# petuum/autodist

Hardware: AMD Instinct MI355X
Metric: images/sec ResNet-50 AllReduce (higher is better)
Workload: dtype bf16; 1 GPU; model=resnet50, global_batch=512, parallelism=dp1, image_size=224

## Files before the change

### autodist_amd/models/resnet.py

```python
import torch
import torch.nn as nn


def _make_bn(ch, fused, relu):
    if fused:
        from autodist_amd.ops.fused_bn import FusedBatchNorm2d
        return FusedBatchNorm2d(ch, relu=relu)
    return nn.BatchNorm2d(ch)


class Bottleneck(nn.Module):
    expansion = 4

    def __init__(self, in_ch, width, stride=1, downsample=None, fused=False):
        super().__init__()
        out_ch = width * self.expansion
        self.fused = fused
        self.conv1 = nn.Conv2d(in_ch, width, 1, bias=False)
        self.bn1 = _make_bn(width, fused, relu=True)
        self.conv2 = nn.Conv2d(width, width, 3, stride=stride, padding=1,
                               bias=False)
        self.bn2 = _make_bn(width, fused, relu=True)
        self.conv3 = nn.Conv2d(width, out_ch, 1, bias=False)
        self.bn3 = _make_bn(out_ch, fused, relu=True)
        self.relu = nn.ReLU(inplace=True)
        self.downsample = downsample

    def forward(self, x):
        if self.fused:
            out = self.bn1(self.conv1(x))
            out = self.bn2(self.conv2(out))
            z = self.conv3(out)
            identity = x if self.downsample is None else self.downsample(x)
            return self.bn3.forward_add(z, identity)
        identity = x
        out = self.relu(self.bn1(self.conv1(x)))
        out = self.relu(self.bn2(self.conv2(out)))
        out = self.bn3(self.conv3(out))
        if self.downsample is not None:
            identity = self.downsample(x)
        return self.relu(out + identity)


class BasicBlock(nn.Module):
    expansion = 1

    def __init__(self, in_ch, width, stride=1, downsample=None, fused=False):
        super().__init__()
        self.fused = fused
        self.conv1 = nn.Conv2d(in_ch, width, 3, stride=stride, padding=1,
                               bias=False)
        self.bn1 = _make_bn(width, fused, relu=True)
        self.conv2 = nn.Conv2d(width, width, 3, padding=1, bias=False)
        self.bn2 = _make_bn(width, fused, relu=True)
        self.relu = nn.ReLU(inplace=True)
        self.downsample = downsample

    def forward(self, x):
        if self.fused:
            out = self.bn1(self.conv1(x))
            z = self.conv2(out)
            identity = x if self.downsample is None else self.downsample(x)
            return self.bn2.forward_add(z, identity)
        identity = x
        out = self.relu(self.bn1(self.conv1(x)))
        out = self.bn2(self.conv2(out))
        if self.downsample is not None:
            identity = self.downsample(x)
        return self.relu(out + identity)


class ResNet(nn.Module):
    def __init__(self, block, layers, num_classes=1000, fused=False):
        super().__init__()
        self.in_ch = 64
        self.fused = fused
        self.conv1 = nn.Conv2d(3, 64, 7, stride=2, padding=3, bias=False)
        self.bn1 = _make_bn(64, fused, relu=True)
# ... 17 lines not shown
    def _make_layer(self, block, width, blocks, stride=1):
        downsample = None
        out_ch = width * block.expansion
        if stride != 1 or self.in_ch != out_ch:
            downsample = nn.Sequential(
                nn.Conv2d(self.in_ch, out_ch, 1, stride=stride, bias=False),
                _make_bn(out_ch, self.fused, relu=False))
        layers = [block(self.in_ch, width, stride, downsample,
                        fused=self.fused)]
        self.in_ch = out_ch
        for _ in range(1, blocks):
            layers.append(block(self.in_ch, width, fused=self.fused))
        return nn.Sequential(*layers)

    def forward(self, x):
        x = self.bn1(self.conv1(x))
        if not self.fused:
            x = self.relu(x)
        x = self.maxpool(x)
        x = self.layer4(self.layer3(self.layer2(self.layer1(x))))
        x = self.avgpool(x).flatten(1)
        return self.fc(x)


def resnet18(num_classes=1000, fused=False):
    return ResNet(BasicBlock, [2, 2, 2, 2], num_classes, fused=fused)


def resnet50(num_classes=1000, fused=False):
    return ResNet(Bottleneck, [3, 4, 6, 3], num_classes, fused=fused)


def resnet101(num_classes=1000, fused=False):
    return ResNet(Bottleneck, [3, 4, 23, 3], num_classes, fused=fused)
# ... 1 lines not shown
```

### autodist_amd/ops/csrc/bn_ops.hip

```cpp
#include "common.h"

#define BN_VEC 8
#define BN_RED_U 4
#define BN_FIN_U 8
#define BN_RELU_NONE 0
#define BN_RELU_Y 1
#define BN_RELU_MASK 2

__device__ __forceinline__ void load8(const __hip_bfloat16* p, float* v) {
  const __hip_bfloat162* p2 = reinterpret_cast<const __hip_bfloat162*>(p);
  float2 a = __bfloat1622float2(p2[0]);
  float2 b = __bfloat1622float2(p2[1]);
  float2 c = __bfloat1622float2(p2[2]);
  float2 d = __bfloat1622float2(p2[3]);
  v[0] = a.x; v[1] = a.y; v[2] = b.x; v[3] = b.y;
  v[4] = c.x; v[5] = c.y; v[6] = d.x; v[7] = d.y;
}
__device__ __forceinline__ void store8(__hip_bfloat16* p, const float* v) {
  __hip_bfloat162* p2 = reinterpret_cast<__hip_bfloat162*>(p);
  p2[0] = __float22bfloat162_rn({v[0], v[1]});
  p2[1] = __float22bfloat162_rn({v[2], v[3]});
  p2[2] = __float22bfloat162_rn({v[4], v[5]});
  p2[3] = __float22bfloat162_rn({v[6], v[7]});
}
// ... 43 lines not shown
                                        float* v) {
  const unsigned w[4] = {r.a.x, r.a.y, r.a.z, r.a.w};
#pragma unroll
  for (int j = 0; j < 4; ++j) {
    v[2 * j] = __uint_as_float(w[j] << 16);
    v[2 * j + 1] = __uint_as_float(w[j] & 0xffff0000u);
  }
}
__device__ __forceinline__ void unpack8(const Raw8<float>& r, float* v) {
  v[0] = r.a.x; v[1] = r.a.y; v[2] = r.a.z; v[3] = r.a.w;
  v[4] = r.b.x; v[5] = r.b.y; v[6] = r.b.z; v[7] = r.b.w;
}
__device__ __forceinline__ void apply_mask8(unsigned bits, float* dv) {
#pragma unroll
  for (int k = 0; k < BN_VEC; ++k) dv[k] = (bits >> k) & 1u ? dv[k] : 0.f;
}

template <typename T>
__global__ void __launch_bounds__(BLOCK_THREADS)
bn_fwd_reduce_kernel(const T* __restrict__ x, float* __restrict__ partial_sum,
                     float* __restrict__ partial_sq, long M, int C) {
#pragma clang fp contract(off)
  int tx_count = min(C / BN_VEC, (int)blockDim.x);
  int tx = threadIdx.x % tx_count;
  int ty = threadIdx.x / tx_count;
  int rows_per_blk = blockDim.x / tx_count;
  int c0 = (blockIdx.y * tx_count + tx) * BN_VEC;
  if (c0 >= C) return;
  float s[BN_VEC] = {0}, q[BN_VEC] = {0};
  const long stride = (long)gridDim.x * rows_per_blk;
// ... 134 lines not shown
#pragma unroll
      for (int k = 0; k < BN_VEC; ++k) v[k] += r[k];
    }
    if (RELU) {
#pragma unroll
      for (int k = 0; k < BN_VEC; ++k) v[k] = fmaxf(v[k], 0.f);
    }
    if (MASK)
      mask[m * (C / BN_VEC) + c0 / BN_VEC] =
          (unsigned char)store8_mask(y + m * C + c0, v);
    else
      store8(y + m * C + c0, v);
  }
}

template <typename T, int RELU>
__device__ __forceinline__ void bn_load_dz(const T* __restrict__ dy,
                                           const T* __restrict__ y,
                                           const unsigned char* __restrict__ mask,
                                           long m, int C, int c0, float* dv) {
  load8(dy + m * C + c0, dv);
  if (RELU == BN_RELU_Y) {
    float yv[BN_VEC];
    load8(y + m * C + c0, yv);
#pragma unroll
    for (int k = 0; k < BN_VEC; ++k) dv[k] = yv[k] > 0.f ? dv[k] : 0.f;
  }
  if (RELU == BN_RELU_MASK)
    apply_mask8(mask[m * (C / BN_VEC) + c0 / BN_VEC], dv);
}

template <typename T, int RELU>
__global__ void __launch_bounds__(BLOCK_THREADS)
bn_bwd_reduce_kernel(const T* __restrict__ x, const T* __restrict__ dy,
                     const T* __restrict__ y,
                     const unsigned char* __restrict__ mask,
                     const float* __restrict__ save_mean,
                     const float* __restrict__ save_rstd,
                     float* __restrict__ partial_dz,
                     float* __restrict__ partial_dzxh, long M, int C) {
#pragma clang fp contract(off)
  int tx_count = min(C / BN_VEC, (int)blockDim.x);
  int tx = threadIdx.x % tx_count;
  int ty = threadIdx.x / tx_count;
  int rows_per_blk = blockDim.x / tx_count;
  int c0 = (blockIdx.y * tx_count + tx) * BN_VEC;
  if (c0 >= C) return;
  float mean[BN_VEC], rstd[BN_VEC];
  load8(save_mean + c0, mean);
  load8(save_rstd + c0, rstd);
  float s[BN_VEC] = {0}, t[BN_VEC] = {0};
  const long stride = (long)gridDim.x * rows_per_blk;
  long m = (long)blockIdx.x * rows_per_blk + ty;
  for (; m + (BN_RED_U - 1) * stride < M; m += BN_RED_U * stride) {
    Raw8<T> rx[BN_RED_U], rd[BN_RED_U], ry[BN_RED_U];
    unsigned rm[BN_RED_U];
#pragma unroll
    for (int u = 0; u < BN_RED_U; ++u) {
      const long mu = m + u * stride;
      rx[u] = load8raw(x + mu * C + c0);
      rd[u] = load8raw(dy + mu * C + c0);
      if (RELU == BN_RELU_Y) ry[u] = load8raw(y + mu * C + c0);
      if (RELU == BN_RELU_MASK) rm[u] = mask[mu * (C / BN_VEC) + c0 / BN_VEC];
    }
    __builtin_amdgcn_sched_barrier(0);
#pragma unroll
    for (int u = 0; u < BN_RED_U; ++u) {
      float xv[BN_VEC], dv[BN_VEC];
      unpack8(rx[u], xv);
      unpack8(rd[u], dv);
      if (RELU == BN_RELU_Y) {
        float yv[BN_VEC];
        unpack8(ry[u], yv);
#pragma unroll
        for (int k = 0; k < BN_VEC; ++k) dv[k] = yv[k] > 0.f ? dv[k] : 0.f;
      }
      if (RELU == BN_RELU_MASK) apply_mask8(rm[u], dv);
#pragma unroll
      for (int k = 0; k < BN_VEC; ++k) {
        s[k] += dv[k];
        t[k] = fmaf(dv[k] * (xv[k] - mean[k]), rstd[k], t[k]);
      }
    }
  }
  for (; m < M; m += stride) {
    float xv[BN_VEC], dv[BN_VEC];
    load8(x + m * C + c0, xv);
    bn_load_dz<T, RELU>(dy, y, mask, m, C, c0, dv);
#pragma unroll
    for (int k = 0; k < BN_VEC; ++k) {
      s[k] += dv[k];
      t[k] = fmaf(dv[k] * (xv[k] - mean[k]), rstd[k], t[k]);
    }
  }
  __shared__ float ls[BLOCK_THREADS * BN_VEC];
  __shared__ float lt[BLOCK_THREADS * BN_VEC];
#pragma unroll
  for (int k = 0; k < BN_VEC; ++k) {
    ls[threadIdx.x * BN_VEC + k] = s[k];
    lt[threadIdx.x * BN_VEC + k] = t[k];
  }
  __syncthreads();
  if (ty == 0) {
// ... 40 lines not shown
  dweight[c] = sdzxh;
  dbias[c] = sdz;
}

template <typename T, int RELU, bool ADD>
__global__ void bn_bwd_apply_kernel(const T* __restrict__ x,
                                    const T* __restrict__ dy,
                                    const T* __restrict__ y,
                                    const unsigned char* __restrict__ mask,
                                    const float* __restrict__ save_mean,
                                    const float* __restrict__ save_rstd,
                                    const float* __restrict__ k1,
                                    const float* __restrict__ k2,
                                    const float* __restrict__ k3,
                                    T* __restrict__ dx, T* __restrict__ dres,
                                    long M, int C) {
  int tx_count = min(C / BN_VEC, (int)blockDim.x);
  int tx = threadIdx.x % tx_count;
  int ty = threadIdx.x / tx_count;
  int rows_per_blk = blockDim.x / tx_count;
  int c0 = (blockIdx.y * tx_count + tx) * BN_VEC;
  if (c0 >= C) return;
  float mean[BN_VEC], rstd[BN_VEC], a1[BN_VEC], a2[BN_VEC], a3[BN_VEC];
  load8(save_mean + c0, mean);
  load8(save_rstd + c0, rstd);
  load8(k1 + c0, a1);
  load8(k2 + c0, a2);
  load8(k3 + c0, a3);
  for (long m = (long)blockIdx.x * rows_per_blk + ty; m < M;
       m += (long)gridDim.x * rows_per_blk) {
    float xv[BN_VEC], dv[BN_VEC];
    load8(x + m * C + c0, xv);
    bn_load_dz<T, RELU>(dy, y, mask, m, C, c0, dv);
    if (ADD) store8(dres + m * C + c0, dv);
    float o[BN_VEC];
#pragma unroll
    for (int k = 0; k < BN_VEC; ++k) {
      float xhat = (xv[k] - mean[k]) * rstd[k];
      o[k] = a1[k] * (dv[k] - a2[k] - xhat * a3[k]);
    }
    store8(dx + m * C + c0, o);
  }
}
```

### autodist_amd/ops/csrc/ext.hip

```cpp
#include <torch/extension.h>
#include <ATen/cuda/CUDAContext.h>

#include "multi_tensor.hip"
#include "bn_ops.hip"
#include "psgd_gemm.hip"
#include "mfma_probe.hip"
#include "attention.hip"
#include "attention_bwd.hip"
#include "ln_ops.hip"
#include "ce_ops.hip"

namespace {

inline hipStream_t cur_stream() {
  return at::cuda::getCurrentCUDAStream().stream();
}

struct BNGeom {
  long M;
  int C;
  int tx_count, rows_per_blk, grid_c;
};

BNGeom bn_geom(const torch::Tensor& x) {
// ... 32 lines not shown
T* bn_ptr(const torch::Tensor& t) {
  return reinterpret_cast<T*>(t.data_ptr());
}

template <typename T, bool RELU, bool ADD, bool MASK>
void bn_launch_fwd_apply(dim3 grid, hipStream_t st, const torch::Tensor& x,
                         const torch::Tensor* res, torch::Tensor& y,
                         unsigned char* mask, const float* scale,
                         const float* shift, const BNGeom& g) {
  hipLaunchKernelGGL((bn_fwd_apply_kernel<T, RELU, ADD, MASK>), grid,
                     dim3(BLOCK_THREADS), 0, st, bn_ptr<const T>(x),
                     ADD ? bn_ptr<const T>(*res) : (const T*)nullptr,
                     bn_ptr<T>(y), mask, scale, shift, g.M, g.C);
}

template <typename T>
std::vector<torch::Tensor> bn_fwd_impl(
    const torch::Tensor& x, const torch::Tensor& weight,
    const torch::Tensor& bias, torch::Tensor& running_mean,
    torch::Tensor& running_var, const c10::optional<torch::Tensor>& res,
    double eps, double momentum, bool relu,
    const c10::optional<torch::Tensor>& ws, bool with_mask) {
  TORCH_CHECK(!with_mask || relu, "the mask is the ReLU mask: relu must be set");
  auto g = bn_geom(x);
  auto fopt = weight.options().dtype(torch::kFloat32);
  torch::Tensor w6 = ws.has_value() ? *ws
      : torch::empty({2 * BN_GM_MAX + 4, (long)g.C}, fopt);
  TORCH_CHECK(w6.size(0) >= 2 * BN_GM_MAX + 4 && w6.size(1) == g.C &&
              w6.is_contiguous());
  float* wp = w6.data_ptr<float>();
  float* partial_sum = wp;
  float* partial_sq = wp + (long)BN_GM_MAX * g.C;
  auto stats = torch::empty({2, (long)g.C}, fopt);
  auto save_mean = stats[0];
  auto save_rstd = stats[1];
  torch::Tensor mask;
  if (with_mask)
    mask = torch::empty({g.M, (long)(g.C / BN_VEC)},
                        x.options().dtype(torch::kUInt8));
  unsigned char* mp = with_mask ? mask.data_ptr<unsigned char>() : nullptr;
  const float* scale = wp + (long)(2 * BN_GM_MAX + 2) * g.C;
  const float* shift = wp + (long)(2 * BN_GM_MAX + 3) * g.C;
  auto y = torch::empty_like(x);
  int gm = bn_reduce_gm(g);
  dim3 grid_r(gm, g.grid_c);
  dim3 grid_a(bn_grid_m(g, 4096), g.grid_c);
  auto st = cur_stream();

  hipLaunchKernelGGL((bn_fwd_reduce_kernel<T>), grid_r, dim3(BLOCK_THREADS),
                     0, st, bn_ptr<const T>(x), partial_sum, partial_sq, g.M,
                     g.C);
  hipLaunchKernelGGL(bn_fwd_finalize_kernel,
                     dim3((g.C + FIN_CH - 1) / FIN_CH),
                     dim3(FIN_CH * FIN_LANES), 0, st, partial_sum, partial_sq,
                     gm, weight.data_ptr<float>(), bias.data_ptr<float>(),
                     running_mean.data_ptr<float>(),
                     running_var.data_ptr<float>(),
                     save_mean.data_ptr<float>(), save_rstd.data_ptr<float>(),
                     const_cast<float*>(scale), const_cast<float*>(shift),
                     g.M, g.C, (float)eps, (float)momentum);
  const torch::Tensor* rp = res.has_value() ? &*res : nullptr;
#define BN_FWD_APPLY(RELU, ADD, MASK)                                        \
  bn_launch_fwd_apply<T, RELU, ADD, MASK>(grid_a, st, x, rp, y, mp, scale,  \
                                          shift, g)
  if (rp) {
    if (with_mask) BN_FWD_APPLY(true, true, true);
    else if (relu) BN_FWD_APPLY(true, true, false);
    else BN_FWD_APPLY(false, true, false);
  } else {
    if (with_mask) BN_FWD_APPLY(true, false, true);
    else if (relu) BN_FWD_APPLY(true, false, false);
    else BN_FWD_APPLY(false, false, false);
  }
#undef BN_FWD_APPLY
  if (with_mask) return {y, save_mean, save_rstd, mask};
// ... 22 lines not shown
                                        c10::optional<torch::Tensor> res,
                                        double eps, double momentum,
                                        bool relu,
                                        c10::optional<torch::Tensor> ws) {
  return bn_fwd_dispatch(x, weight, bias, running_mean, running_var, res, eps,
                         momentum, relu, ws, false);
}

std::vector<torch::Tensor> bn_fwd_train_mask(
    torch::Tensor x, torch::Tensor weight, torch::Tensor bias,
    torch::Tensor running_mean, torch::Tensor running_var,
    c10::optional<torch::Tensor> res, double eps, double momentum, bool relu,
    c10::optional<torch::Tensor> ws) {
  return bn_fwd_dispatch(x, weight, bias, running_mean, running_var, res, eps,
                         momentum, relu, ws, true);
}

template <typename T, int RELU>
std::vector<torch::Tensor> bn_bwd_impl(
    const torch::Tensor& x, const torch::Tensor& dy, const torch::Tensor& yq,
    const torch::Tensor& save_mean, const torch::Tensor& save_rstd,
    const torch::Tensor& weight, bool need_dres,
    const c10::optional<torch::Tensor>& ws) {
  auto g = bn_geom(x);
  auto fopt = weight.options().dtype(torch::kFloat32);
  torch::Tensor w5 = ws.has_value() ? *ws
      : torch::empty({2 * BN_GM_MAX + 3, (long)g.C}, fopt);
  TORCH_CHECK(w5.size(0) >= 2 * BN_GM_MAX + 3 && w5.size(1) == g.C &&
              w5.is_contiguous());
  const T* yp = nullptr;
// ... 16 lines not shown
  auto dweight = torch::empty({g.C}, fopt);
  auto dbias = torch::empty({g.C}, fopt);
  auto dx = torch::empty_like(x);
  torch::Tensor dres;
  if (need_dres) dres = torch::empty_like(x);
  dim3 block(BLOCK_THREADS);
  int gm = bn_reduce_gm(g);
  dim3 grid_r(gm, g.grid_c);
  dim3 grid_a(bn_grid_m(g, 4096), g.grid_c);
  auto st = cur_stream();
  const float* sm = save_mean.data_ptr<float>();
  const float* sr = save_rstd.data_ptr<float>();

  hipLaunchKernelGGL((bn_bwd_reduce_kernel<T, RELU>), grid_r, block, 0, st,
                     bn_ptr<const T>(x), bn_ptr<const T>(dy), yp, mp, sm, sr,
                     partial_dz, partial_dzxh, g.M, g.C);
  hipLaunchKernelGGL(bn_bwd_finalize_kernel,
                     dim3((g.C + FIN_CH - 1) / FIN_CH),
                     dim3(FIN_CH * FIN_LANES), 0, st, partial_dz,
                     partial_dzxh, gm, weight.data_ptr<float>(), sr, k1, k2,
                     k3, dweight.data_ptr<float>(), dbias.data_ptr<float>(),
                     g.M, g.C);
  if (need_dres)
    hipLaunchKernelGGL((bn_bwd_apply_kernel<T, RELU, true>), grid_a, block, 0,
                       st, bn_ptr<const T>(x), bn_ptr<const T>(dy), yp, mp,
                       sm, sr, k1, k2, k3, bn_ptr<T>(dx), bn_ptr<T>(dres),
                       g.M, g.C);
  else
    hipLaunchKernelGGL((bn_bwd_apply_kernel<T, RELU, false>), grid_a, block,
                       0, st, bn_ptr<const T>(x), bn_ptr<const T>(dy), yp, mp,
                       sm, sr, k1, k2, k3, bn_ptr<T>(dx), (T*)nullptr, g.M,
                       g.C);
  std::vector<torch::Tensor> out = {dx, dweight, dbias};
  if (need_dres) out.push_back(dres);
  return out;
}

template <int RELU>
std::vector<torch::Tensor> bn_bwd_dispatch(
    const torch::Tensor& x, const torch::Tensor& dy, const torch::Tensor& yq,
    const torch::Tensor& save_mean, const torch::Tensor& save_rstd,
    const torch::Tensor& weight, bool need_dres,
    const c10::optional<torch::Tensor>& ws) {
  if (x.scalar_type() == torch::kBFloat16)
    return bn_bwd_impl<__hip_bfloat16, RELU>(x, dy, yq, save_mean, save_rstd,
                                             weight, need_dres, ws);
  TORCH_CHECK(x.scalar_type() == torch::kFloat32);
// ... 12 lines not shown
                                      need_dres, ws);
  return bn_bwd_dispatch<BN_RELU_NONE>(x, dy, y, save_mean, save_rstd, weight,
                                       need_dres, ws);
}

std::vector<torch::Tensor> bn_bwd_mask(torch::Tensor x, torch::Tensor dy,
                                       torch::Tensor mask,
                                       torch::Tensor save_mean,
                                       torch::Tensor save_rstd,
                                       torch::Tensor weight, bool relu,
                                       bool need_dres,
                                       c10::optional<torch::Tensor> ws) {
  TORCH_CHECK(relu, "the mask is the ReLU mask: relu must be set");
  return bn_bwd_dispatch<BN_RELU_MASK>(x, dy, mask, save_mean, save_rstd,
                                       weight, need_dres, ws);
}

void check_f32_flat(const torch::Tensor& t, const char* name) {
  TORCH_CHECK(t.is_cuda(), name, " must be on GPU");
  TORCH_CHECK(t.is_contiguous(), name, " must be contiguous");
  TORCH_CHECK(t.scalar_type() == torch::kFloat32, name, " must be fp32");
}

template <typename GT>
void launch_fused_sgd(torch::Tensor& p, const GT* g,
                      c10::optional<torch::Tensor>& buf, double lr,
                      double momentum, double dampening, double weight_decay,
                      bool nesterov, bool first_step, bool maximize) {
  long n = p.numel();
  dim3 grid(grid_for(n)), block(BLOCK_THREADS);
// ... 656 lines not shown
  m.def("scatter_add_rows", &scatter_add_rows, "rowwise scatter-add");
  m.def("gather_rows", &gather_rows, "rowwise gather");
  m.def("sparse_apply_rows", &sparse_apply_rows,
        "fused row-wise SGD/Adagrad/Adam update of unique rows (gfx950)");
  m.def("bn_fwd_train", &bn_fwd_train,
        "fused NHWC batchnorm fwd (+add+relu), returns y/save_mean/save_rstd");
  m.def("bn_bwd", &bn_bwd,
        "fused NHWC batchnorm bwd (+relu-mask+dres), returns "
        "dx/dweight/dbias[/dres]");
  m.def("bn_fwd_train_mask", &bn_fwd_train_mask,
        "bn_fwd_train with relu that also returns the bit-packed ReLU mask "
        "[M, C/8] uint8");
  m.def("bn_bwd_mask", &bn_bwd_mask,
        "bn_bwd that takes the packed mask of bn_fwd_train_mask in place of "
        "y");
  m.attr("BN_RED_U") = BN_RED_U;
  m.attr("BN_FIN_U") = BN_FIN_U;
  m.def("psgd_mq", &psgd_mq, "PowerSGD P = M @ Q (MFMA f32 16x16x4)");
  m.def("psgd_mtp", &psgd_mtp, "PowerSGD Qn = M^T @ P (MFMA f32 16x16x4)");
  m.def("psgd_decompress_ef", &psgd_decompress_ef,
        "fused hat = P Q^T * scale; err = M - hat; flat = hat");
  m.def("psgd_add_err_pad", &psgd_add_err_pad,
        "padded M = flat + err (zero tail)");
  m.def("mfma_probe", &mfma_probe,
        "diagnostic: v_mfma_f32_16x16x32_bf16 A/B layout probe");
  m.def("ce_fwd", &ce_fwd,
        "fused online-softmax cross-entropy fwd -> loss_rows, m, l2s");
  m.def("ce_bwd", &ce_bwd, "fused cross-entropy bwd -> dlogits (bf16)");
  m.def("col_sum", &col_sum, "bf16 [N,H] column sum -> fp32 [H]");
  m.def("ln_fwd", &ln_fwd,
// ... 18 lines not shown
```

### autodist_amd/ops/fused_bn.py

```python
from typing import Optional

import torch

from autodist_amd.ops import api as ops_api


class _FusedBNFunction(torch.autograd.Function):
    @staticmethod
    def forward(ctx, x, weight, bias, running_mean, running_var,
                momentum, eps, relu, residual, ws=None):
        use_hip = x.is_cuda and ops_api.has_gpu_ops()
        ctx.ws_bwd = ws[1] if ws is not None else None
        if use_hip and relu:
            y, save_mean, save_rstd, sign = ops_api.ext().bn_fwd_train_mask(
                x, weight, bias, running_mean, running_var, residual,
                eps, momentum, relu, ws[0] if ws is not None else None)
        elif use_hip:
            y, save_mean, save_rstd = ops_api.ext().bn_fwd_train(
                x, weight, bias, running_mean, running_var, residual,
                eps, momentum, relu, ws[0] if ws is not None else None)
            sign = y
        else:
            xf = x.float()
            m = xf.numel() // xf.size(1)
# ... 31 lines not shown
                weight, relu, has_res, ctx.ws_bwd)
            dx, dweight, dbias = out[0], out[1], out[2]
            dres = out[3] if has_res else None
        else:
            dyf = dy.float()
            if relu:
                dyf = dyf * (sign > 0).float()
            dres = dyf.to(dy.dtype) if has_res else None
            dxf, dweight, dbias = torch.ops.aten.native_batch_norm_backward(
                dyf, x.float(), weight, None, None, save_mean, save_rstd,
                True, 0.0, [True, True, True])
            dx = dxf.to(x.dtype)
        return (dx, dweight, dbias, None, None, None, None, None, dres, None)


def fused_bn_train(x, weight, bias, running_mean, running_var,
                   momentum=0.1, eps=1e-5, relu=False,
                   residual: Optional[torch.Tensor] = None, ws=None):
    return _FusedBNFunction.apply(x, weight, bias, running_mean, running_var,
                                  momentum, eps, relu, residual, ws)


class FusedBatchNorm2d(torch.nn.Module):

    def __init__(self, num_features, eps=1e-5, momentum=0.1, relu=False):
        super().__init__()
        self.num_features = num_features
        self.eps = eps
        self.momentum = momentum
        self.relu = relu
        self.weight = torch.nn.Parameter(torch.ones(num_features))
        self.bias = torch.nn.Parameter(torch.zeros(num_features))
        self.register_buffer("running_mean", torch.zeros(num_features))
        self.register_buffer("running_var", torch.ones(num_features))
        self.register_buffer("num_batches_tracked",
                             torch.tensor(0, dtype=torch.long))
        self._ws = None

    def _check(self, x):
        if x.is_cuda and not x.is_contiguous(memory_format=torch.channels_last):
            x = x.contiguous(memory_format=torch.channels_last)
        return x

    def forward(self, x, residual: Optional[torch.Tensor] = None):
        x = self._check(x)
        if residual is not None:
            residual = self._check(residual)
        if self.training:
            self.num_batches_tracked += 1
            if x.is_cuda and (self._ws is None
                              or self._ws[0].device != x.device):
                self._ws = (
                    torch.empty(2 * 512 + 4, self.num_features,
                                device=x.device),
                    torch.empty(2 * 512 + 3, self.num_features,
                                device=x.device))
            return fused_bn_train(x, self.weight, self.bias,
                                  self.running_mean, self.running_var,
                                  self.momentum, self.eps, self.relu, residual,
                                  ws=self._ws if x.is_cuda else None)
        scale = self.weight * (self.running_var + self.eps).rsqrt()
        shift = self.bias - self.running_mean * scale
        y = x * scale[None, :, None, None].to(x.dtype) + \
            shift[None, :, None, None].to(x.dtype)
        if residual is not None:
            y = y + residual
        return torch.relu(y) if self.relu else y

    def forward_add(self, x, residual):
        return self.forward(x, residual)

    def extra_repr(self):
        return f"{self.num_features}, relu={self.relu}"
```

Before: 9384 images/sec.

## Fuse stem BN+ReLU+maxpool and downsample BN into residual BN apply

Adds a fused kernel for the stem that applies BN, ReLU and the 3x3 stride-2 max-pool in one pass, storing packed argmax words instead of the full-resolution activation. The backward pass recomputes the pooled gradient scatter inside the BN backward reduce and apply kernels. It also fuses the downsample-branch BN into the residual-add BN apply, so the downsample BN output is never materialized. This cuts full-size activation writes and reads and some launches, at the cost of more complex gather logic and bf16 rounding-order subtleties.

New measurement: 9898 images/sec (median of 6 runs). +5.5%, better.

```diff
diff --git a/autodist_amd/models/resnet.py b/autodist_amd/models/resnet.py
--- a/autodist_amd/models/resnet.py
+++ b/autodist_amd/models/resnet.py
@@ -31,8 +31,10 @@
             out = self.bn1(self.conv1(x))
             out = self.bn2(self.conv2(out))
             z = self.conv3(out)
-            identity = x if self.downsample is None else self.downsample(x)
-            return self.bn3.forward_add(z, identity)
+            if self.downsample is None:
+                return self.bn3.forward_add(z, x)
+            return self.bn3.forward_add_bn(z, self.downsample[0](x),
+                                           self.downsample[1])
         identity = x
         out = self.relu(self.bn1(self.conv1(x)))
         out = self.relu(self.bn2(self.conv2(out)))
@@ -60,8 +62,10 @@
         if self.fused:
             out = self.bn1(self.conv1(x))
             z = self.conv2(out)
-            identity = x if self.downsample is None else self.downsample(x)
-            return self.bn2.forward_add(z, identity)
+            if self.downsample is None:
+                return self.bn2.forward_add(z, x)
+            return self.bn2.forward_add_bn(z, self.downsample[0](x),
+                                           self.downsample[1])
         identity = x
         out = self.relu(self.bn1(self.conv1(x)))
         out = self.bn2(self.conv2(out))
@@ -109,10 +113,10 @@
         return nn.Sequential(*layers)
 
     def forward(self, x):
-        x = self.bn1(self.conv1(x))
-        if not self.fused:
-            x = self.relu(x)
-        x = self.maxpool(x)
+        if self.fused:
+            x = self.bn1.forward_pool(self.conv1(x))
+        else:
+            x = self.maxpool(self.relu(self.bn1(self.conv1(x))))
         x = self.layer4(self.layer3(self.layer2(self.layer1(x))))
         x = self.avgpool(x).flatten(1)
         return self.fc(x)
diff --git a/autodist_amd/ops/csrc/bn_ops.hip b/autodist_amd/ops/csrc/bn_ops.hip
--- a/autodist_amd/ops/csrc/bn_ops.hip
+++ b/autodist_amd/ops/csrc/bn_ops.hip
@@ -81,6 +81,65 @@
 __device__ __forceinline__ void apply_mask8(unsigned bits, float* dv) {
 #pragma unroll
   for (int k = 0; k < BN_VEC; ++k) dv[k] = (bits >> k) & 1u ? dv[k] : 0.f;
+}
+
+__device__ __forceinline__ float round_to(float v, const __hip_bfloat16*) {
+  return __bfloat162float(__float2bfloat16(v));
+}
+__device__ __forceinline__ float round_to(float v, const float*) { return v; }
+
+#define BN_RELU_POOL 3
+#define BN_POOL_NONE 15u
+#define BN_POOL_NEVER 14u
+struct BNPool {
+  const unsigned* amax;
+  int H, W, Ho, Wo;
+};
+template <typename T>
+struct PoolTaps {
+  Raw8<T> d[4];
+  unsigned a[4];
+  unsigned codes;
+};
+template <typename T>
+__device__ __forceinline__ void pool_issue(const T* __restrict__ dy,
+                                           const BNPool& p, long m, int C,
+                                           int c0, PoolTaps<T>& t) {
+  const unsigned mm = (unsigned)m;
+  const unsigned q = mm / (unsigned)p.W;
+  const int w = (int)(mm - q * (unsigned)p.W);
+  const unsigned n = q / (unsigned)p.H;
+  const int h = (int)(q - n * (unsigned)p.H);
+  const int ho = h >> 1, wo = w >> 1;
+  const bool hb = (h & 1) && ho + 1 < p.Ho;
+  const bool wb = (w & 1) && wo + 1 < p.Wo;
+  const unsigned kh = 1 + (h & 1), kw = 1 + (w & 1);
+  const unsigned o0 = ((n * p.Ho + ho) * p.Wo + wo) * C + c0;
+  const unsigned dh = hb ? p.Wo * C : 0, dw = wb ? C : 0;
+  const unsigned o[4] = {o0, o0 + dw, o0 + dh, o0 + dh + dw};
+  t.codes = (kh * 3 + kw) | (wb ? kh * 3 : BN_POOL_NEVER) << 8 |
+            (hb ? kw : BN_POOL_NEVER) << 16 |
+            (hb && wb ? 0u : BN_POOL_NEVER) << 24;
+#pragma unroll
+  for (int j = 0; j < 4; ++j) {
+    t.d[j] = load8raw(dy + o[j]);
+    t.a[j] = p.amax[o[j] / BN_VEC];
+  }
+}
+template <typename T>
+__device__ __forceinline__ void pool_dz(const PoolTaps<T>& t, float* dv) {
+  float acc[BN_VEC] = {0};
+#pragma unroll
+  for (int j = 0; j < 4; ++j) {
+    float d[BN_VEC];
+    unpack8(t.d[j], d);
+    const unsigned e = t.a[j] ^ (((t.codes >> (8 * j)) & 15u) * 0x11111111u);
+#pragma unroll
+    for (int k = 0; k < BN_VEC; ++k)
+      acc[k] += ((e >> (4 * k)) & 15u) == 0u ? d[k] : 0.f;
+  }
+#pragma unroll
+  for (int k = 0; k < BN_VEC; ++k) dv[k] = round_to(acc[k], (const T*)nullptr);
 }
 
 template <typename T>
@@ -245,11 +304,115 @@
   }
 }
 
+template <typename T>
+__global__ void bn_fwd_pool_apply_kernel(const T* __restrict__ x,
+                                         T* __restrict__ y,
+                                         unsigned* __restrict__ amax,
+                                         const float* __restrict__ scale,
+                                         const float* __restrict__ shift,
+                                         BNPool p, long Mo, int C) {
+  int tx_count = min(C / BN_VEC, (int)blockDim.x);
+  int tx = threadIdx.x % tx_count;
+  int ty = threadIdx.x / tx_count;
+  int rows_per_blk = blockDim.x / tx_count;
+  int c0 = (blockIdx.y * tx_count + tx) * BN_VEC;
+  if (c0 >= C) return;
+  float sc[BN_VEC], sh[BN_VEC];
+  load8(scale + c0, sc);
+  load8(shift + c0, sh);
+  for (long mo = (long)blockIdx.x * rows_per_blk + ty; mo < Mo;
+       mo += (long)gridDim.x * rows_per_blk) {
+    const unsigned mm = (unsigned)mo;
+    const unsigned q = mm / (unsigned)p.Wo;
+    const int wo = (int)(mm - q * (unsigned)p.Wo);
+    const unsigned n = q / (unsigned)p.Ho;
+    const int ho = (int)(q - n * (unsigned)p.Ho);
+    Raw8<T> rx[9];
+    bool ok[9];
+#pragma unroll
+    for (int kh = 0; kh < 3; ++kh) {
+      const int h = 2 * ho - 1 + kh;
+      const int hc = min(max(h, 0), p.H - 1);
+#pragma unroll
+      for (int kw = 0; kw < 3; ++kw) {
+        const int w = 2 * wo - 1 + kw;
+        const int wc = min(max(w, 0), p.W - 1);
+        ok[kh * 3 + kw] = h == hc && w == wc;
+        rx[kh * 3 + kw] =
+            load8raw(x + (((long)n * p.H + hc) * p.W + wc) * C + c0);
+      }
+    }
+    float best[BN_VEC];
+    unsigned idx[BN_VEC];
+#pragma unroll
+    for (int k = 0; k < BN_VEC; ++k) { best[k] = -1.f; idx[k] = 0; }
+#pragma unroll
+    for (int j = 0; j < 9; ++j) {
+      float v[BN_VEC];
+      unpack8(rx[j], v);
+#pragma unroll
+      for (int k = 0; k < BN_VEC; ++k) {
+        float r = round_to(fmaxf(fmaf(v[k], sc[k], sh[k]), 0.f),
+                           (const T*)nullptr);
+        const bool take = ok[j] && r > best[k];
+        best[k] = take ? r : best[k];
+        idx[k] = take ? (unsigned)j : idx[k];
+      }
+    }
+    unsigned word = 0;
+#pragma unroll
+    for (int k = 0; k < BN_VEC; ++k)
+      word |= (best[k] > 0.f ? idx[k] : BN_POOL_NONE) << (4 * k);
+    store8(y + mo * C + c0, best);
+    amax[mo * (C / BN_VEC) + c0 / BN_VEC] = word;
+  }
+}
+
+template <typename T>
+__global__ void bn_fwd_apply_add_bn_kernel(
+    const T* __restrict__ z, const T* __restrict__ zd, T* __restrict__ y,
+    unsigned char* __restrict__ mask, const float* __restrict__ scale,
+    const float* __restrict__ shift, const float* __restrict__ scale_d,
+    const float* __restrict__ shift_d, long M, int C) {
+  int tx_count = min(C / BN_VEC, (int)blockDim.x);
+  int tx = threadIdx.x % tx_count;
+  int ty = threadIdx.x / tx_count;
+  int rows_per_blk = blockDim.x / tx_count;
+  int c0 = (blockIdx.y * tx_count + tx) * BN_VEC;
+  if (c0 >= C) return;
+  float sc[BN_VEC], sh[BN_VEC], scd[BN_VEC], shd[BN_VEC];
+  load8(scale + c0, sc);
+  load8(shift + c0, sh);
+  load8(scale_d + c0, scd);
+  load8(shift_d + c0, shd);
+  for (long m = (long)blockIdx.x * rows_per_blk + ty; m < M;
+       m += (long)gridDim.x * rows_per_blk) {
+    float v[BN_VEC], r[BN_VEC];
+    load8(z + m * C + c0, v);
+    load8(zd + m * C + c0, r);
+#pragma unroll
+    for (int k = 0; k < BN_VEC; ++k) {
+      v[k] = fmaf(v[k], sc[k], sh[k]);
+      v[k] += round_to(fmaf(r[k], scd[k], shd[k]), (const T*)nullptr);
+      v[k] = fmaxf(v[k], 0.f);
+    }
+    mask[m * (C / BN_VEC) + c0 / BN_VEC] =
+        (unsigned char)store8_mask(y + m * C + c0, v);
+  }
+}
+
 template <typename T, int RELU>
 __device__ __forceinline__ void bn_load_dz(const T* __restrict__ dy,
                                            const T* __restrict__ y,
                                            const unsigned char* __restrict__ mask,
-                                           long m, int C, int c0, float* dv) {
+                                           const BNPool& pool, long m, int C,
+                                           int c0, float* dv) {
+  if (RELU == BN_RELU_POOL) {
+    PoolTaps<T> t;
+    pool_issue(dy, pool, m, C, c0, t);
+    pool_dz(t, dv);
+    return;
+  }
   load8(dy + m * C + c0, dv);
   if (RELU == BN_RELU_Y) {
     float yv[BN_VEC];
@@ -263,13 +426,15 @@
 
 template <typename T, int RELU>
 __global__ void __launch_bounds__(BLOCK_THREADS)
+__attribute__((amdgpu_waves_per_eu(RELU == BN_RELU_POOL ? 2 : 1)))
 bn_bwd_reduce_kernel(const T* __restrict__ x, const T* __restrict__ dy,
                      const T* __restrict__ y,
                      const unsigned char* __restrict__ mask,
                      const float* __restrict__ save_mean,
                      const float* __restrict__ save_rstd,
                      float* __restrict__ partial_dz,
-                     float* __restrict__ partial_dzxh, long M, int C) {
+                     float* __restrict__ partial_dzxh, long M, int C,
+                     BNPool pool) {
 #pragma clang fp contract(off)
   int tx_count = min(C / BN_VEC, (int)blockDim.x);
   int tx = threadIdx.x % tx_count;
@@ -286,11 +451,17 @@
   for (; m + (BN_RED_U - 1) * stride < M; m += BN_RED_U * stride) {
     Raw8<T> rx[BN_RED_U], rd[BN_RED_U], ry[BN_RED_U];
     unsigned rm[BN_RED_U];
+    PoolTaps<T> rp[BN_RED_U];
 #pragma unroll
     for (int u = 0; u < BN_RED_U; ++u) {
       const long mu = m + u * stride;
       rx[u] = load8raw(x + mu * C + c0);
-      rd[u] = load8raw(dy + mu * C + c0);
+      if (RELU == BN_RELU_POOL) {
+        pool_issue(dy, pool, mu, C, c0, rp[u]);
+        __builtin_amdgcn_sched_barrier(0);
+      } else {
+        rd[u] = load8raw(dy + mu * C + c0);
+      }
       if (RELU == BN_RELU_Y) ry[u] = load8raw(y + mu * C + c0);
       if (RELU == BN_RELU_MASK) rm[u] = mask[mu * (C / BN_VEC) + c0 / BN_VEC];
     }
@@ -299,7 +470,8 @@
     for (int u = 0; u < BN_RED_U; ++u) {
       float xv[BN_VEC], dv[BN_VEC];
       unpack8(rx[u], xv);
-      unpack8(rd[u], dv);
+      if (RELU == BN_RELU_POOL) pool_dz(rp[u], dv);
+      else unpack8(rd[u], dv);
       if (RELU == BN_RELU_Y) {
         float yv[BN_VEC];
         unpack8(ry[u], yv);
@@ -312,12 +484,13 @@
         s[k] += dv[k];
         t[k] = fmaf(dv[k] * (xv[k] - mean[k]), rstd[k], t[k]);
       }
+      if (RELU == BN_RELU_POOL) __builtin_amdgcn_sched_barrier(0);
     }
   }
   for (; m < M; m += stride) {
     float xv[BN_VEC], dv[BN_VEC];
     load8(x + m * C + c0, xv);
-    bn_load_dz<T, RELU>(dy, y, mask, m, C, c0, dv);
+    bn_load_dz<T, RELU>(dy, y, mask, pool, m, C, c0, dv);
 #pragma unroll
     for (int k = 0; k < BN_VEC; ++k) {
       s[k] += dv[k];
@@ -388,7 +561,7 @@
                                     const float* __restrict__ k2,
                                     const float* __restrict__ k3,
                                     T* __restrict__ dx, T* __restrict__ dres,
-                                    long M, int C) {
+                                    long M, int C, BNPool pool) {
   int tx_count = min(C / BN_VEC, (int)blockDim.x);
   int tx = threadIdx.x % tx_count;
   int ty = threadIdx.x / tx_count;
@@ -405,7 +578,7 @@
        m += (long)gridDim.x * rows_per_blk) {
     float xv[BN_VEC], dv[BN_VEC];
     load8(x + m * C + c0, xv);
-    bn_load_dz<T, RELU>(dy, y, mask, m, C, c0, dv);
+    bn_load_dz<T, RELU>(dy, y, mask, pool, m, C, c0, dv);
     if (ADD) store8(dres + m * C + c0, dv);
     float o[BN_VEC];
 #pragma unroll
diff --git a/autodist_amd/ops/csrc/ext.hip b/autodist_amd/ops/csrc/ext.hip
--- a/autodist_amd/ops/csrc/ext.hip
+++ b/autodist_amd/ops/csrc/ext.hip
@@ -70,15 +70,19 @@
                      bn_ptr<T>(y), mask, scale, shift, g.M, g.C);
 }
 
+struct BNStats {
+  torch::Tensor save_mean, save_rstd;
+  const float* scale;
+  const float* shift;
+  torch::Tensor ws;
+};
+
 template <typename T>
-std::vector<torch::Tensor> bn_fwd_impl(
-    const torch::Tensor& x, const torch::Tensor& weight,
-    const torch::Tensor& bias, torch::Tensor& running_mean,
-    torch::Tensor& running_var, const c10::optional<torch::Tensor>& res,
-    double eps, double momentum, bool relu,
-    const c10::optional<torch::Tensor>& ws, bool with_mask) {
-  TORCH_CHECK(!with_mask || relu, "the mask is the ReLU mask: relu must be set");
-  auto g = bn_geom(x);
+BNStats bn_fwd_stats(const torch::Tensor& x, const BNGeom& g,
+                     const torch::Tensor& weight, const torch::Tensor& bias,
+                     torch::Tensor& running_mean, torch::Tensor& running_var,
+                     double eps, double momentum,
+                     const c10::optional<torch::Tensor>& ws) {
   auto fopt = weight.options().dtype(torch::kFloat32);
   torch::Tensor w6 = ws.has_value() ? *ws
       : torch::empty({2 * BN_GM_MAX + 4, (long)g.C}, fopt);
@@ -90,17 +94,10 @@
   auto stats = torch::empty({2, (long)g.C}, fopt);
   auto save_mean = stats[0];
   auto save_rstd = stats[1];
-  torch::Tensor mask;
-  if (with_mask)
-    mask = torch::empty({g.M, (long)(g.C / BN_VEC)},
-                        x.options().dtype(torch::kUInt8));
-  unsigned char* mp = with_mask ? mask.data_ptr<unsigned char>() : nullptr;
   const float* scale = wp + (long)(2 * BN_GM_MAX + 2) * g.C;
   const float* shift = wp + (long)(2 * BN_GM_MAX + 3) * g.C;
-  auto y = torch::empty_like(x);
   int gm = bn_reduce_gm(g);
   dim3 grid_r(gm, g.grid_c);
-  dim3 grid_a(bn_grid_m(g, 4096), g.grid_c);
   auto st = cur_stream();
 
   hipLaunchKernelGGL((bn_fwd_reduce_kernel<T>), grid_r, dim3(BLOCK_THREADS),
@@ -115,6 +112,31 @@
                      save_mean.data_ptr<float>(), save_rstd.data_ptr<float>(),
                      const_cast<float*>(scale), const_cast<float*>(shift),
                      g.M, g.C, (float)eps, (float)momentum);
+  return {save_mean, save_rstd, scale, shift, w6};
+}
+
+template <typename T>
+std::vector<torch::Tensor> bn_fwd_impl(
+    const torch::Tensor& x, const torch::Tensor& weight,
+    const torch::Tensor& bias, torch::Tensor& running_mean,
+    torch::Tensor& running_var, const c10::optional<torch::Tensor>& res,
+    double eps, double momentum, bool relu,
+    const c10::optional<torch::Tensor>& ws, bool with_mask) {
+  TORCH_CHECK(!with_mask || relu, "the mask is the ReLU mask: relu must be set");
+  auto g = bn_geom(x);
+  BNStats s = bn_fwd_stats<T>(x, g, weight, bias, running_mean, running_var,
+                              eps, momentum, ws);
+  auto save_mean = s.save_mean, save_rstd = s.save_rstd;
+  const float* scale = s.scale;
+  const float* shift = s.shift;
+  torch::Tensor mask;
+  if (with_mask)
+    mask = torch::empty({g.M, (long)(g.C / BN_VEC)},
+                        x.options().dtype(torch::kUInt8));
+  unsigned char* mp = with_mask ? mask.data_ptr<unsigned char>() : nullptr;
+  auto y = torch::empty_like(x);
+  dim3 grid_a(bn_grid_m(g, 4096), g.grid_c);
+  auto st = cur_stream();
   const torch::Tensor* rp = res.has_value() ? &*res : nullptr;
 #define BN_FWD_APPLY(RELU, ADD, MASK)                                        \
   bn_launch_fwd_apply<T, RELU, ADD, MASK>(grid_a, st, x, rp, y, mp, scale,  \
@@ -167,6 +189,107 @@
     c10::optional<torch::Tensor> ws) {
   return bn_fwd_dispatch(x, weight, bias, running_mean, running_var, res, eps,
                          momentum, relu, ws, true);
+}
+
+inline BNPool bn_pool_geom(const torch::Tensor& x, const BNGeom& g) {
+  BNPool p;
+  p.amax = nullptr;
+  p.H = (int)x.size(2);
+  p.W = (int)x.size(3);
+  p.Ho = (p.H - 1) / 2 + 1;
+  p.Wo = (p.W - 1) / 2 + 1;
+  TORCH_CHECK(g.M < (1L << 31), "bn pool: N*H*W must be below 2^31");
+  TORCH_CHECK(x.size(0) * (long)p.Ho * p.Wo * g.C < (1L << 31),
+              "bn pool: the pooled tensor must hold fewer than 2^31 elements");
+  return p;
+}
+
+template <typename T>
+std::vector<torch::Tensor> bn_fwd_pool_impl(
+    const torch::Tensor& x, const torch::Tensor& weight,
+    const torch::Tensor& bias, torch::Tensor& running_mean,
+    torch::Tensor& running_var, double eps, double momentum,
+    const c10::optional<torch::Tensor>& ws) {
+  auto g = bn_geom(x);
+  BNPool p = bn_pool_geom(x, g);
+  BNStats s = bn_fwd_stats<T>(x, g, weight, bias, running_mean, running_var,
+                              eps, momentum, ws);
+  BNGeom go = g;
+  go.M = x.size(0) * (long)p.Ho * p.Wo;
+  auto y = torch::empty({x.size(0), x.size(1), (long)p.Ho, (long)p.Wo},
+                        x.options().memory_format(at::MemoryFormat::ChannelsLast));
+  auto amax = torch::empty({go.M, (long)(g.C / BN_VEC)},
+                           x.options().dtype(torch::kInt32));
+  dim3 grid_a(bn_grid_m(go, 4096), g.grid_c);
+  hipLaunchKernelGGL((bn_fwd_pool_apply_kernel<T>), grid_a,
+                     dim3(BLOCK_THREADS), 0, cur_stream(), bn_ptr<const T>(x),
+                     bn_ptr<T>(y), bn_ptr<unsigned>(amax), s.scale, s.shift,
+                     p, go.M, g.C);
+  return {y, s.save_mean, s.save_rstd, amax};
+}
+
+std::vector<torch::Tensor> bn_fwd_train_pool(
+    torch::Tensor x, torch::Tensor weight, torch::Tensor bias,
+    torch::Tensor running_mean, torch::Tensor running_var, double eps,
+    double momentum, c10::optional<torch::Tensor> ws) {
+  if (x.scalar_type() == torch::kBFloat16)
+    return bn_fwd_pool_impl<__hip_bfloat16>(x, weight, bias, running_mean,
+                                            running_var, eps, momentum, ws);
+  TORCH_CHECK(x.scalar_type() == torch::kFloat32);
+  return bn_fwd_pool_impl<float>(x, weight, bias, running_mean, running_var,
+                                 eps, momentum, ws);
+}
+
+template <typename T>
+std::vector<torch::Tensor> bn_fwd_add_bn_impl(
+    const torch::Tensor& z, const torch::Tensor& zd,
+    const torch::Tensor& weight, const torch::Tensor& bias,
+    torch::Tensor& running_mean, torch::Tensor& running_var, double eps,
+    double momentum, const c10::optional<torch::Tensor>& ws,
+    const torch::Tensor& weight_d, const torch::Tensor& bias_d,
+    torch::Tensor& running_mean_d, torch::Tensor& running_var_d, double eps_d,
+    double momentum_d, const c10::optional<torch::Tensor>& ws_d) {
+  auto g = bn_geom(z);
+  auto gd = bn_geom(zd);
+  TORCH_CHECK(zd.sizes() == z.sizes() && zd.scalar_type() == z.scalar_type() &&
+                  zd.device() == z.device() && gd.M == g.M,
+              "bn_fwd_train_add_bn: z and zd must agree in shape and dtype");
+  TORCH_CHECK(!ws.has_value() || !ws_d.has_value() ||
+                  ws->data_ptr() != ws_d->data_ptr(),
+              "bn_fwd_train_add_bn: the two BNs need workspaces of their own");
+  BNStats s = bn_fwd_stats<T>(z, g, weight, bias, running_mean, running_var,
+                              eps, momentum, ws);
+  BNStats sd = bn_fwd_stats<T>(zd, gd, weight_d, bias_d, running_mean_d,
+                               running_var_d, eps_d, momentum_d, ws_d);
+  auto y = torch::empty_like(z);
+  auto mask = torch::empty({g.M, (long)(g.C / BN_VEC)},
+                           z.options().dtype(torch::kUInt8));
+  dim3 grid_a(bn_grid_m(g, 4096), g.grid_c);
+  hipLaunchKernelGGL((bn_fwd_apply_add_bn_kernel<T>), grid_a,
+                     dim3(BLOCK_THREADS), 0, cur_stream(), bn_ptr<const T>(z),
+                     bn_ptr<const T>(zd), bn_ptr<T>(y),
+                     mask.data_ptr<unsigned char>(), s.scale, s.shift,
+                     sd.scale, sd.shift, g.M, g.C);
+  return {y, mask, s.save_mean, s.save_rstd, sd.save_mean, sd.save_rstd};
+}
+
+std::vector<torch::Tensor> bn_fwd_train_add_bn(
+    torch::Tensor z, torch::Tensor zd, torch::Tensor weight,
+    torch::Tensor bias, torch::Tensor running_mean, torch::Tensor running_var,
+    double eps, double momentum, c10::optional<torch::Tensor> ws,
+    torch::Tensor weight_d, torch::Tensor bias_d, torch::Tensor running_mean_d,
+    torch::Tensor running_var_d, double eps_d, double momentum_d,
+    c10::optional<torch::Tensor> ws_d) {
+  if (z.scalar_type() == torch::kBFloat16)
+    return bn_fwd_add_bn_impl<__hip_bfloat16>(
+        z, zd, weight, bias, running_mean, running_var, eps, momentum, ws,
+        weight_d, bias_d, running_mean_d, running_var_d, eps_d, momentum_d,
+        ws_d);
+  TORCH_CHECK(z.scalar_type() == torch::kFloat32);
+  return bn_fwd_add_bn_impl<float>(
+      z, zd, weight, bias, running_mean, running_var, eps, momentum, ws,
+      weight_d, bias_d, running_mean_d, running_var_d, eps_d, momentum_d,
+      ws_d);
 }
 
 template <typename T, int RELU>
@@ -213,7 +336,7 @@
 
   hipLaunchKernelGGL((bn_bwd_reduce_kernel<T, RELU>), grid_r, block, 0, st,
                      bn_ptr<const T>(x), bn_ptr<const T>(dy), yp, mp, sm, sr,
-                     partial_dz, partial_dzxh, g.M, g.C);
+                     partial_dz, partial_dzxh, g.M, g.C, BNPool{});
   hipLaunchKernelGGL(bn_bwd_finalize_kernel,
                      dim3((g.C + FIN_CH - 1) / FIN_CH),
                      dim3(FIN_CH * FIN_LANES), 0, st, partial_dz,
@@ -224,12 +347,12 @@
     hipLaunchKernelGGL((bn_bwd_apply_kernel<T, RELU, true>), grid_a, block, 0,
                        st, bn_ptr<const T>(x), bn_ptr<const T>(dy), yp, mp,
                        sm, sr, k1, k2, k3, bn_ptr<T>(dx), bn_ptr<T>(dres),
-                       g.M, g.C);
+                       g.M, g.C, BNPool{});
   else
     hipLaunchKernelGGL((bn_bwd_apply_kernel<T, RELU, false>), grid_a, block,
                        0, st, bn_ptr<const T>(x), bn_ptr<const T>(dy), yp, mp,
                        sm, sr, k1, k2, k3, bn_ptr<T>(dx), (T*)nullptr, g.M,
-                       g.C);
+                       g.C, BNPool{});
   std::vector<torch::Tensor> out = {dx, dweight, dbias};
   if (need_dres) out.push_back(dres);
   return out;
@@ -272,6 +395,81 @@
   TORCH_CHECK(relu, "the mask is the ReLU mask: relu must be set");
   return bn_bwd_dispatch<BN_RELU_MASK>(x, dy, mask, save_mean, save_rstd,
                                        weight, need_dres, ws);
+}
+
+template <typename T>
+std::vector<torch::Tensor> bn_bwd_pool_impl(
+    const torch::Tensor& x, const torch::Tensor& dy,
+    const torch::Tensor& argmax, const torch::Tensor& save_mean,
+    const torch::Tensor& save_rstd, const torch::Tensor& weight,
+    const c10::optional<torch::Tensor>& ws) {
+  auto g = bn_geom(x);
+  BNPool p = bn_pool_geom(x, g);
+  const long Mo = x.size(0) * (long)p.Ho * p.Wo;
+  TORCH_CHECK(dy.dim() == 4 && dy.size(0) == x.size(0) && dy.size(1) == g.C &&
+                  dy.size(2) == p.Ho && dy.size(3) == p.Wo &&
+                  dy.scalar_type() == x.scalar_type() &&
+                  dy.device() == x.device() &&
+                  dy.is_contiguous(at::MemoryFormat::ChannelsLast),
+              "dy must be the channels_last [N, C, Ho, Wo] gradient of the "
+              "pooled y");
+  TORCH_CHECK(argmax.scalar_type() == torch::kInt32 && argmax.is_contiguous() &&
+                  argmax.dim() == 2 && argmax.size(0) == Mo &&
+                  argmax.size(1) == g.C / BN_VEC &&
+                  argmax.device() == x.device(),
+              "argmax must be the [N*Ho*Wo, C/8] int32 tensor of "
+              "bn_fwd_train_pool");
+  p.amax = bn_ptr<const unsigned>(argmax);
+  auto fopt = weight.options().dtype(torch::kFloat32);
+  torch::Tensor w5 = ws.has_value() ? *ws
+      : torch::empty({2 * BN_GM_MAX + 3, (long)g.C}, fopt);
+  TORCH_CHECK(w5.size(0) >= 2 * BN_GM_MAX + 3 && w5.size(1) == g.C &&
+              w5.is_contiguous());
+  float* wp = w5.data_ptr<float>();
+  float* partial_dz = wp;
+  float* partial_dzxh = wp + (long)BN_GM_MAX * g.C;
+  float* k1 = wp + (long)(2 * BN_GM_MAX + 0) * g.C;
+  float* k2 = wp + (long)(2 * BN_GM_MAX + 1) * g.C;
+  float* k3 = wp + (long)(2 * BN_GM_MAX + 2) * g.C;
+  auto dweight = torch::empty({g.C}, fopt);
+  auto dbias = torch::empty({g.C}, fopt);
+  auto dx = torch::empty_like(x);
+  dim3 block(BLOCK_THREADS);
+  int gm = bn_reduce_gm(g);
+  dim3 grid_r(gm, g.grid_c);
+  dim3 grid_a(bn_grid_m(g, 4096), g.grid_c);
+  auto st = cur_stream();
+  const float* sm = save_mean.data_ptr<float>();
+  const float* sr = save_rstd.data_ptr<float>();
+  hipLaunchKernelGGL((bn_bwd_reduce_kernel<T, BN_RELU_POOL>), grid_r, block, 0,
+                     st, bn_ptr<const T>(x), bn_ptr<const T>(dy),
+                     (const T*)nullptr, (const unsigned char*)nullptr, sm, sr,
+                     partial_dz, partial_dzxh, g.M, g.C, p);
+  hipLaunchKernelGGL(bn_bwd_finalize_kernel,
+                     dim3((g.C + FIN_CH - 1) / FIN_CH),
+                     dim3(FIN_CH * FIN_LANES), 0, st, partial_dz,
+                     partial_dzxh, gm, weight.data_ptr<float>(), sr, k1, k2,
+                     k3, dweight.data_ptr<float>(), dbias.data_ptr<float>(),
+                     g.M, g.C);
+  hipLaunchKernelGGL((bn_bwd_apply_kernel<T, BN_RELU_POOL, false>), grid_a,
+                     block, 0, st, bn_ptr<const T>(x), bn_ptr<const T>(dy),
+                     (const T*)nullptr, (const unsigned char*)nullptr, sm, sr,
+                     k1, k2, k3, bn_ptr<T>(dx), (T*)nullptr, g.M, g.C, p);
+  return {dx, dweight, dbias};
+}
+
+std::vector<torch::Tensor> bn_bwd_pool(torch::Tensor x, torch::Tensor dy,
+                                       torch::Tensor argmax,
+                                       torch::Tensor save_mean,
+                                       torch::Tensor save_rstd,
+                                       torch::Tensor weight,
+                                       c10::optional<torch::Tensor> ws) {
+  if (x.scalar_type() == torch::kBFloat16)
+    return bn_bwd_pool_impl<__hip_bfloat16>(x, dy, argmax, save_mean,
+                                            save_rstd, weight, ws);
+  TORCH_CHECK(x.scalar_type() == torch::kFloat32);
+  return bn_bwd_pool_impl<float>(x, dy, argmax, save_mean, save_rstd, weight,
+                                 ws);
 }
 
 void check_f32_flat(const torch::Tensor& t, const char* name) {
@@ -958,6 +1156,17 @@
   m.def("bn_bwd_mask", &bn_bwd_mask,
         "bn_bwd that takes the packed mask of bn_fwd_train_mask in place of "
         "y");
+  m.def("bn_fwd_train_pool", &bn_fwd_train_pool,
+        "bn + relu + 3x3/stride 2/pad 1 max-pool: (x, weight, bias, "
+        "running_mean, running_var, eps, momentum, ws) -> (pooled y, "
+        "save_mean, save_rstd, argmax words)");
+  m.def("bn_bwd_pool", &bn_bwd_pool,
+        "backward of bn_fwd_train_pool: (x, dy_pooled, argmax, save_mean, "
+        "save_rstd, weight, ws) -> (dx, dweight, dbias)");
+  m.def("bn_fwd_train_add_bn", &bn_fwd_train_add_bn,
+        "relu(bn(z) + bn_d(zd)): (z, zd, then weight, bias, running_mean, "
+        "running_var, eps, momentum, ws of each BN) -> (y, mask, save_mean, "
+        "save_rstd, save_mean_d, save_rstd_d)");
   m.attr("BN_RED_U") = BN_RED_U;
   m.attr("BN_FIN_U") = BN_FIN_U;
   m.def("psgd_mq", &psgd_mq, "PowerSGD P = M @ Q (MFMA f32 16x16x4)");
diff --git a/autodist_amd/ops/fused_bn.py b/autodist_amd/ops/fused_bn.py
--- a/autodist_amd/ops/fused_bn.py
+++ b/autodist_amd/ops/fused_bn.py
@@ -3,6 +3,9 @@
 import torch
 
 from autodist_amd.ops import api as ops_api
+
+
+SPLIT_PATH = False
 
 
 class _FusedBNFunction(torch.autograd.Function):
@@ -69,6 +72,56 @@
         return (dx, dweight, dbias, None, None, None, None, None, dres, None)
 
 
+class _FusedBNPoolFunction(torch.autograd.Function):
+
+    @staticmethod
+    def forward(ctx, x, weight, bias, running_mean, running_var, momentum,
+                eps, ws):
+        y, save_mean, save_rstd, argmax = ops_api.ext().bn_fwd_train_pool(
+            x, weight, bias, running_mean, running_var, eps, momentum,
+            ws[0] if ws is not None else None)
+        ctx.ws_bwd = ws[1] if ws is not None else None
+        ctx.save_for_backward(x, argmax, save_mean, save_rstd, weight)
+        return y
+
+    @staticmethod
+    def backward(ctx, dy):
+        x, argmax, save_mean, save_rstd, weight = ctx.saved_tensors
+        dx, dweight, dbias = ops_api.ext().bn_bwd_pool(
+            x, dy.contiguous(memory_format=torch.channels_last), argmax,
+            save_mean, save_rstd, weight, ctx.ws_bwd)
+        return dx, dweight, dbias, None, None, None, None, None
+
+
+class _FusedBNAddBNFunction(torch.autograd.Function):
+
+    @staticmethod
+    def forward(ctx, z, zd, weight, bias, running_mean, running_var, momentum,
+                eps, ws, weight_d, bias_d, running_mean_d, running_var_d,
+                momentum_d, eps_d, ws_d):
+        y, mask, sm, sr, sm_d, sr_d = ops_api.ext().bn_fwd_train_add_bn(
+            z, zd, weight, bias, running_mean, running_var, eps, momentum,
+            ws[0] if ws is not None else None,
+            weight_d, bias_d, running_mean_d, running_var_d, eps_d,
+            momentum_d, ws_d[0] if ws_d is not None else None)
+        ctx.ws_bwd = ws[1] if ws is not None else None
+        ctx.ws_bwd_d = ws_d[1] if ws_d is not None else None
+        ctx.save_for_backward(z, zd, mask, sm, sr, sm_d, sr_d, weight,
+                              weight_d)
+        return y
+
+    @staticmethod
+    def backward(ctx, dy):
+        z, zd, mask, sm, sr, sm_d, sr_d, weight, weight_d = ctx.saved_tensors
+        dy = dy.contiguous(memory_format=torch.channels_last)
+        bwd = ops_api.ext().bn_bwd_mask
+        dz, dw, db = bwd(z, dy, mask, sm, sr, weight, True, False, ctx.ws_bwd)
+        dzd, dw_d, db_d = bwd(zd, dy, mask, sm_d, sr_d, weight_d, True, False,
+                              ctx.ws_bwd_d)
+        return (dz, dzd, dw, db, None, None, None, None, None,
+                dw_d, db_d, None, None, None, None, None)
+
+
 def fused_bn_train(x, weight, bias, running_mean, running_var,
                    momentum=0.1, eps=1e-5, relu=False,
                    residual: Optional[torch.Tensor] = None, ws=None):
@@ -97,23 +150,25 @@
             x = x.contiguous(memory_format=torch.channels_last)
         return x
 
+    def _workspace(self, x):
+        if not x.is_cuda:
+            return None
+        if self._ws is None or self._ws[0].device != x.device:
+            self._ws = (
+                torch.empty(2 * 512 + 4, self.num_features, device=x.device),
+                torch.empty(2 * 512 + 3, self.num_features, device=x.device))
+        return self._ws
+
     def forward(self, x, residual: Optional[torch.Tensor] = None):
         x = self._check(x)
         if residual is not None:
             residual = self._check(residual)
         if self.training:
             self.num_batches_tracked += 1
-            if x.is_cuda and (self._ws is None
-                              or self._ws[0].device != x.device):
-                self._ws = (
-                    torch.empty(2 * 512 + 4, self.num_features,
-                                device=x.device),
-                    torch.empty(2 * 512 + 3, self.num_features,
-                                device=x.device))
             return fused_bn_train(x, self.weight, self.bias,
                                   self.running_mean, self.running_var,
                                   self.momentum, self.eps, self.relu, residual,
-                                  ws=self._ws if x.is_cuda else None)
+                                  ws=self._workspace(x))
         scale = self.weight * (self.running_var + self.eps).rsqrt()
         shift = self.bias - self.running_mean * scale
         y = x * scale[None, :, None, None].to(x.dtype) + \
@@ -125,5 +180,34 @@
     def forward_add(self, x, residual):
         return self.forward(x, residual)
 
+    def _fused_kernels(self, x):
+        return (self.training and x.is_cuda and ops_api.has_gpu_ops()
+                and not SPLIT_PATH)
+
+    def forward_pool(self, x):
+        assert self.relu, "forward_pool is bn -> relu -> max-pool"
+        if not self._fused_kernels(x):
+            return torch.nn.functional.max_pool2d(self.forward(x), 3, 2, 1)
+        x = self._check(x)
+        self.num_batches_tracked += 1
+        return _FusedBNPoolFunction.apply(
+            x, self.weight, self.bias, self.running_mean, self.running_var,
+            self.momentum, self.eps, self._workspace(x))
+
+    def forward_add_bn(self, z, zd, other_bn):
+        if not (self._fused_kernels(z) and self.relu
+                and isinstance(other_bn, FusedBatchNorm2d)
+                and other_bn.training and not other_bn.relu):
+            return self.forward_add(z, other_bn(zd))
+        z, zd = self._check(z), other_bn._check(zd)
+        self.num_batches_tracked += 1
+        other_bn.num_batches_tracked += 1
+        return _FusedBNAddBNFunction.apply(
+            z, zd, self.weight, self.bias, self.running_mean,
+            self.running_var, self.momentum, self.eps, self._workspace(z),
+            other_bn.weight, other_bn.bias, other_bn.running_mean,
+            other_bn.running_var, other_bn.momentum, other_bn.eps,
+            other_bn._workspace(zd))
+
     def extra_repr(self):
         return f"{self.num_features}, relu={self.relu}"
```
